# zrlhahaha/Direct12PBRRenderer

Hardware: AMD Instinct MI355X
Metric: shaded Mpixel/s at 4K G-buffer (full deferred frame: clustered shade + bloom + auto-exposure + ACES) (higher is better)
Workload: dtype f32

## Files before the change

direct12pbrrenderer_amd/csrc/exposure.hip:

```cpp
#include "pbr_internal.hpp"
#include "pbr_device.hpp"

using namespace pbr;

__device__ __forceinline__ uint32_t luminance_bin(float r, float g, float b, float min_log, float inv_range) {
#pragma clang fp contract(off)
    const float lum = (r * 0.2126f + g * 0.7152f) + b * 0.0722f;
    if (lum < EPSILON_F) return 0u;
    const float l = saturatef((log2f(lum) - min_log) * inv_range);
    return (uint32_t)floorf(l * 254.0f + 1.0f);
}

constexpr int HIST_BLOCKS = 512, HIST_NT = 1024, HIST_NW = HIST_NT / 64;

__global__ __launch_bounds__(HIST_NT) void k_lum_histogram(const pbr_half* __restrict__ hdr, uint32_t w, uint32_t h, uint32_t pitch,
                                                             float min_log, float inv_range, uint32_t* __restrict__ hist, bool vec2) {
    __shared__ uint32_t sh[HIST_NW][PBR_HISTOGRAM_BINS];
    const int wave = threadIdx.x >> 6;
    for (int i = threadIdx.x; i < HIST_NW * PBR_HISTOGRAM_BINS; i += HIST_NT) (&sh[0][0])[i] = 0u;
    __syncthreads();
    uint32_t* my = sh[wave];
    const uint32_t group = threadIdx.x >> 8, gl = threadIdx.x & 255u, stride = gridDim.x * 4u;
    if (vec2) {
        const uint32_t wp = w >> 1, upr = (wp + 255u) >> 8, units = upr * h;
        for (uint32_t u = blockIdx.x * 4u + group; u < units; u += 2 * stride) {
            const uint32_t u2 = u + stride;
            const uint32_t ya = u / upr, xa = (u - ya * upr) * 256u + gl;
            const uint32_t yb = u2 / upr, xb = (u2 - yb * upr) * 256u + gl;
            const bool ina = xa < wp, inb = u2 < units && xb < wp;
            uint4 ra = make_uint4(0u, 0u, 0u, 0u), rb = ra;
            if (ina) ra = *reinterpret_cast<const uint4*>(hdr + 4 * ((size_t)ya * pitch + 2 * xa));
            if (inb) rb = *reinterpret_cast<const uint4*>(hdr + 4 * ((size_t)yb * pitch + 2 * xb));
            const H4 p0 = *reinterpret_cast<const H4*>(&ra.x), p1 = *reinterpret_cast<const H4*>(&ra.z);
            const H4 p2 = *reinterpret_cast<const H4*>(&rb.x), p3 = *reinterpret_cast<const H4*>(&rb.z);
            hist_count(my, luminance_bin((float)p0.x, (float)p0.y, (float)p0.z, min_log, inv_range), ina);
            hist_count(my, luminance_bin((float)p1.x, (float)p1.y, (float)p1.z, min_log, inv_range), ina);
            hist_count(my, luminance_bin((float)p2.x, (float)p2.y, (float)p2.z, min_log, inv_range), inb);
            hist_count(my, luminance_bin((float)p3.x, (float)p3.y, (float)p3.z, min_log, inv_range), inb);
        }
    } else {
        const uint32_t upr = (w + 255u) >> 8, units = upr * h;
        for (uint32_t u = blockIdx.x * 4u + group; u < units; u += stride) {
            const uint32_t y = u / upr, x = (u - y * upr) * 256u + gl;
            const bool in = x < w;
            F4 c = f4(0.0f, 0.0f, 0.0f, 0.0f);
            if (in) c = load_h4(hdr + 4 * ((size_t)y * pitch + x));
            hist_count(my, luminance_bin(c.x, c.y, c.z, min_log, inv_range), in);
        }
    }
    __syncthreads();
    if (threadIdx.x < PBR_HISTOGRAM_BINS) {
        uint32_t s = 0;
#pragma unroll
        for (int k = 0; k < HIST_NW; k++) s += sh[k][threadIdx.x];
        if (s) atomicAdd(&hist[threadIdx.x], s);
    }
}

__device__ __forceinline__ float adapted_luminance(float* sh, const uint32_t* __restrict__ hist, uint32_t pixel_count, float min_log, float range,
                                                   float delta_time, float prev) {
#pragma clang fp contract(off)
    const uint32_t index = threadIdx.x;
    const uint32_t num_pixels = hist[index];
    sh[index] = (float)(uint32_t)(num_pixels * index);
    __syncthreads();
    for (uint32_t step = PBR_HISTOGRAM_BINS >> 1; step > 0; step >>= 1) {
        if (index < step) sh[index] += sh[index + step];
        __syncthreads();
    }
    float result = 0.0f;
    if (index == 0) {
        const float sum_value = sh[0];
        const float average_bin = sum_value / (float)(pixel_count - num_pixels);
        uint32_t bin = (average_bin == average_bin && average_bin > 0.0f)
                           ? (average_bin >= 4294967296.0f ? 0xFFFFFFFFu : (uint32_t)average_bin) : 0u;
        const float log_l = ((float)bin - 1.0f) / 254.0f;
        const float lum = exp2f(log_l * range + min_log);
        const float tt = saturatef(1.0f - expf(-delta_time * 1.6f));
        result = prev + tt * (lum - prev);
    }
    return result;
}

__global__ __launch_bounds__(256) void k_lum_average(uint32_t* __restrict__ hist, uint32_t pixel_count, float min_log, float range,
                                                       float delta_time, float* __restrict__ avg) {
    __shared__ float sh[PBR_HISTOGRAM_BINS];
    const float r = adapted_luminance(sh, hist, pixel_count, min_log, range, delta_time, avg[0]);
    hist[threadIdx.x] = 0u;
    if (threadIdx.x == 0) avg[0] = r;
}

struct AverageViews { uint32_t* hist[PBR_MAX_VIEWS]; float* avg[PBR_MAX_VIEWS]; float delta_time[PBR_MAX_VIEWS]; };
__global__ __launch_bounds__(256) void k_lum_average_views(AverageViews vs, uint32_t pixel_count, float min_log, float range) {
    __shared__ float sh[PBR_HISTOGRAM_BINS];
    uint32_t* hist = vs.hist[blockIdx.x];
    float* avg = vs.avg[blockIdx.x];
    const float r = adapted_luminance(sh, hist, pixel_count, min_log, range, vs.delta_time[blockIdx.x], avg[0]);
    hist[threadIdx.x] = 0u;
    if (threadIdx.x == 0) avg[0] = r;
}

__device__ __forceinline__ float aces1(float x) {
    const float a = 2.51f, b = 0.03f, c = 2.43f, d = 0.59f, e = 0.14f;
    return saturatef((x * (a * x + b)) * rcp(x * (c * x + d) + e));
}
__device__ __forceinline__ uint32_t tonemap_px(float r, float g, float b, float inv_den) {
    const float m[3] = {aces1(r * inv_den), aces1(g * inv_den), aces1(b * inv_den)};
    uint32_t px = 0xFF000000u;
#pragma unroll
    for (int k = 0; k < 3; k++) {
        const float gc = m[k] > 0.0f ? __builtin_amdgcn_exp2f(0.454545f * __builtin_amdgcn_logf(m[k])) : 0.0f;
        px |= (uint32_t)(saturatef(gc) * 255.0f + 0.5f) << (8 * k);
    }
    return px;
}

typedef float tm2 __attribute__((ext_vector_type(2)));
__device__ __forceinline__ tm2 aces2(tm2 x) {
    const float a = 2.51f, b = 0.03f, c = 2.43f, d = 0.59f, e = 0.14f;
    const tm2 num = x * (x * a + b), den = x * (x * c + d) + e;
    tm2 q;
    q.x = saturatef(num.x * rcp(den.x));
    q.y = saturatef(num.y * rcp(den.y));
    return q;
}
__device__ __forceinline__ void tonemap_px2(tm2 r, tm2 g, tm2 b, float inv_den, uint32_t& p0, uint32_t& p1) {
    const tm2 m[3] = {aces2(r * inv_den), aces2(g * inv_den), aces2(b * inv_den)};
    p0 = p1 = 0xFF000000u;
#pragma unroll
    for (int k = 0; k < 3; k++) {
        tm2 lg, gc;
        lg.x = __builtin_amdgcn_logf(m[k].x); lg.y = __builtin_amdgcn_logf(m[k].y);
        lg = lg * 0.454545f;
        gc.x = m[k].x > 0.0f ? __builtin_amdgcn_exp2f(lg.x) : 0.0f;
        gc.y = m[k].y > 0.0f ? __builtin_amdgcn_exp2f(lg.y) : 0.0f;
        gc.x = saturatef(gc.x); gc.y = saturatef(gc.y);
        const tm2 v = gc * 255.0f + 0.5f;
        p0 |= (uint32_t)v.x << (8 * k);
        p1 |= (uint32_t)v.y << (8 * k);
    }
}

__device__ __forceinline__ void tonemap_pixels(const pbr_half* __restrict__ hdr, uint32_t w, uint32_t h, uint32_t pitch,
                                               float avg_lum, uint32_t* __restrict__ out, uint32_t out_pitch, bool aligned) {
    const float l_max = 9.6f * avg_lum;
    const float inv_den = 1.0f / (l_max + 0.001f);
    const uint32_t wp = (w + 1) >> 1;
    const uint32_t upr = (wp + 255u) >> 8, units = upr * h;
    for (uint32_t u = blockIdx.x; u < units; u += gridDim.x) {
        const uint32_t y = u / upr, xp = (u - y * upr) * 256u + threadIdx.x;
        if (xp >= wp) continue;
        const uint32_t x = xp * 2;
        if (aligned && x + 1 < w) {
            const uint4 raw = *reinterpret_cast<const uint4*>(hdr + 4 * ((size_t)y * pitch + x));
            const H4 p0 = *reinterpret_cast<const H4*>(&raw.x);
            const H4 p1 = *reinterpret_cast<const H4*>(&raw.z);
            uint2 o;
            tm2 r2, g2, b2;
            r2.x = (float)p0.x; r2.y = (float)p1.x; g2.x = (float)p0.y; g2.y = (float)p1.y; b2.x = (float)p0.z; b2.y = (float)p1.z;
            tonemap_px2(r2, g2, b2, inv_den, o.x, o.y);
            *reinterpret_cast<uint2*>(out + (size_t)y * out_pitch + x) = o;
        } else {
            for (uint32_t xx = x; xx < min(x + 2, w); xx++) {
                const F4 c = load_h4(hdr + 4 * ((size_t)y * pitch + xx));
                out[(size_t)y * out_pitch + xx] = tonemap_px(c.x, c.y, c.z, inv_den);
            }
        }
    }
}

__global__ __launch_bounds__(256) void k_tonemap(const pbr_half* __restrict__ hdr, uint32_t w, uint32_t h, uint32_t pitch,
                                                   const float* __restrict__ avg, uint32_t* __restrict__ out, uint32_t out_pitch, bool aligned) {
    tonemap_pixels(hdr, w, h, pitch, avg[0], out, out_pitch, aligned);
}

struct TonemapViews {
    const pbr_half* hdr[PBR_MAX_VIEWS];
    const float* avg[PBR_MAX_VIEWS];
    uint32_t* out[PBR_MAX_VIEWS];
    uint32_t pitch[PBR_MAX_VIEWS], out_pitch[PBR_MAX_VIEWS];
    bool aligned[PBR_MAX_VIEWS];
};
__global__ __launch_bounds__(256) void k_tonemap_views(TonemapViews vs, uint32_t w, uint32_t h) {
    const uint32_t v = blockIdx.y;
    tonemap_pixels(vs.hdr[v], w, h, vs.pitch[v], vs.avg[v][0], vs.out[v], vs.out_pitch[v], vs.aligned[v]);
}

__global__ __launch_bounds__(256) void k_average_tonemap(const uint32_t* __restrict__ hist, uint32_t pixel_count, float min_log, float range,
                                                           float delta_time, const float* __restrict__ avg_in, float* __restrict__ avg_out,
                                                           uint32_t* __restrict__ hist_clear,
                                                           const pbr_half* __restrict__ hdr, uint32_t w, uint32_t h, uint32_t pitch,
                                                           uint32_t* __restrict__ out, uint32_t out_pitch, bool aligned) {
    __shared__ float sh[PBR_HISTOGRAM_BINS];
    __shared__ float s_avg;
    const float r = adapted_luminance(sh, hist, pixel_count, min_log, range, delta_time, avg_in[0]);
    if (threadIdx.x == 0) s_avg = r;
    if (blockIdx.x == 0) {
        if (hist_clear) hist_clear[threadIdx.x] = 0u;
        if (threadIdx.x == 0) avg_out[0] = r;
    }
    __syncthreads();
    tonemap_pixels(hdr, w, h, pitch, s_avg, out, out_pitch, aligned);
}

static unsigned tonemap_blocks(uint32_t w, uint32_t h) {
    const size_t pairs = (size_t)((w + 1) / 2) * h;
    const unsigned blocks = (unsigned)((pairs + 255) / 256);
    return blocks > 2048 ? 2048 : blocks;
}
static bool tonemap_aligned(const pbr_half* hdr, uint32_t pitch, const uint32_t* rgba8, uint32_t out_pitch) {
    return (((uintptr_t)hdr & 15u) == 0u) && (((uintptr_t)rgba8 & 7u) == 0u) && (((pitch | out_pitch) & 1u) == 0u);
}

extern "C" {

pbr_status pbr_lum_histogram(pbr_ctx* ctx, const pbr_half* hdr, uint32_t w, uint32_t h, uint32_t pitch,
                             float min_log, float inv_range, uint32_t* hist256) {
    if (!ctx) return PBR_ERR_INVALID;
    PBR_REQUIRE(ctx, hdr && hist256, "pbr_lum_histogram: null pointer");
    PBR_REQUIRE(ctx, w && h && w <= 65535 && h <= 65535 && pitch >= w, "pbr_lum_histogram: bad size");
    static const int max_blocks = pbr::knob_int("PBR_HIST_BLOCKS", HIST_BLOCKS);
    size_t n = (size_t)w * h;
    int blocks = (int)((n + 4095) / 4096);
    if (blocks > max_blocks) blocks = max_blocks;
    if (blocks < 1) blocks = 1;
    const bool vec2 = (((uintptr_t)hdr & 15u) == 0u) && (((w | pitch) & 1u) == 0u);
    hipLaunchKernelGGL(k_lum_histogram, dim3(blocks), dim3(HIST_NT), 0, ctx->stream, hdr, w, h, pitch, min_log, inv_range, hist256, vec2);
    return launched(ctx, "k_lum_histogram");
}

pbr_status pbr_lum_average(pbr_ctx* ctx, uint32_t* hist256, uint32_t pixel_count, float min_log, float range,
                           float delta_time, float* avg_inout) {
    if (!ctx) return PBR_ERR_INVALID;
    PBR_REQUIRE(ctx, hist256 && avg_inout, "pbr_lum_average: null pointer");
    hipLaunchKernelGGL(k_lum_average, dim3(1), dim3(256), 0, ctx->stream, hist256, pixel_count, min_log, range, delta_time, avg_inout);
    return launched(ctx, "k_lum_average");
}

pbr_status pbr_tonemap(pbr_ctx* ctx, const pbr_half* hdr, uint32_t w, uint32_t h, uint32_t pitch,
                       const float* avg, uint32_t* rgba8, uint32_t out_pitch) {
    if (!ctx) return PBR_ERR_INVALID;
    PBR_REQUIRE(ctx, hdr && avg && rgba8, "pbr_tonemap: null pointer");
    PBR_REQUIRE(ctx, w && h && w <= 65535 && h <= 65535 && pitch >= w && out_pitch >= w, "pbr_tonemap: bad size");
    hipLaunchKernelGGL(k_tonemap, dim3(tonemap_blocks(w, h)), dim3(256), 0, ctx->stream, hdr, w, h, pitch, avg, rgba8, out_pitch,
                       tonemap_aligned(hdr, pitch, rgba8, out_pitch));
    return launched(ctx, "k_tonemap");
}

pbr_status pbr_average_tonemap(pbr_ctx* ctx, const uint32_t* hist256, uint32_t pixel_count, float min_log, float range, float delta_time,
                               const float* avg_in, float* avg_out, uint32_t* hist_clear256,
                               const pbr_half* hdr, uint32_t w, uint32_t h, uint32_t pitch, uint32_t* rgba8, uint32_t out_pitch) {
    if (!ctx) return PBR_ERR_INVALID;
    PBR_REQUIRE(ctx, hist256 && avg_in && avg_out && hdr && rgba8, "pbr_average_tonemap: null pointer");
    PBR_REQUIRE(ctx, avg_in != avg_out && hist_clear256 != hist256, "pbr_average_tonemap: avg_out must differ from avg_in and hist_clear256 from hist256 (every block reads them)");
    PBR_REQUIRE(ctx, w && h && w <= 65535 && h <= 65535 && pitch >= w && out_pitch >= w, "pbr_average_tonemap: bad size");
    hipLaunchKernelGGL(k_average_tonemap, dim3(tonemap_blocks(w, h)), dim3(256), 0, ctx->stream, hist256, pixel_count, min_log, range, delta_time,
                       avg_in, avg_out, hist_clear256, hdr, w, h, pitch, rgba8, out_pitch, tonemap_aligned(hdr, pitch, rgba8, out_pitch));
    return launched(ctx, "k_average_tonemap");
}

pbr_status pbr_lum_average_views(pbr_ctx* ctx, const pbr_view* views, uint32_t n, uint32_t pixel_count, float min_log, float range) {
    if (!ctx) return PBR_ERR_INVALID;
    PBR_REQUIRE(ctx, views_count_ok(views, n), "pbr_lum_average_views: need 1 .. PBR_MAX_VIEWS views");
    AverageViews vs{};
    for (uint32_t i = 0; i < n; i++) {
        PBR_REQUIRE(ctx, views[i].hist256 && views[i].avg, "pbr_lum_average_views: null pointer");
        vs.hist[i] = views[i].hist256; vs.avg[i] = views[i].avg; vs.delta_time[i] = views[i].g.DeltaTime;
    }
    PBR_REQUIRE(ctx, views_disjoint(views, n, 2, [](const pbr_view& v, int k, uintptr_t& lo, uintptr_t& hi) {
                    if (k == 0) { lo = addr(v.hist256); hi = lo + PBR_HISTOGRAM_BINS * sizeof(uint32_t); }
                    else { lo = addr(v.avg); hi = lo + sizeof(float); } }),
                "pbr_lum_average_views: two views share a histogram or luminance cell");
    hipLaunchKernelGGL(k_lum_average_views, dim3(n), dim3(256), 0, ctx->stream, vs, pixel_count, min_log, range);
    return launched(ctx, "k_lum_average_views");
}

pbr_status pbr_tonemap_views(pbr_ctx* ctx, const pbr_view* views, uint32_t n, uint32_t w, uint32_t h) {
    if (!ctx) return PBR_ERR_INVALID;
    PBR_REQUIRE(ctx, views_count_ok(views, n), "pbr_tonemap_views: need 1 .. PBR_MAX_VIEWS views");
    PBR_REQUIRE(ctx, w && h && w <= 65535 && h <= 65535, "pbr_tonemap_views: bad size");
    TonemapViews vs{};
    for (uint32_t i = 0; i < n; i++) {
        const pbr_view& v = views[i];
        PBR_REQUIRE(ctx, v.hdr && v.avg && v.rgba8, "pbr_tonemap_views: null pointer");
        PBR_REQUIRE(ctx, v.hdr_pitch >= w && v.out_pitch >= w, "pbr_tonemap_views: bad size");
        vs.hdr[i] = v.hdr; vs.avg[i] = v.avg; vs.out[i] = v.rgba8; vs.pitch[i] = v.hdr_pitch; vs.out_pitch[i] = v.out_pitch;
        vs.aligned[i] = tonemap_aligned(v.hdr, v.hdr_pitch, v.rgba8, v.out_pitch);
    }
    PBR_REQUIRE(ctx, views_disjoint(views, n, 1, [&](const pbr_view& v, int, uintptr_t& lo, uintptr_t& hi) {
                    lo = addr(v.rgba8); hi = lo + ((size_t)v.out_pitch * (h - 1) + w) * sizeof(uint32_t); }),
                "pbr_tonemap_views: two views share an LDR target");
    hipLaunchKernelGGL(k_tonemap_views, dim3(tonemap_blocks(w, h), n), dim3(256), 0, ctx->stream, vs, w, h);
    return launched(ctx, "k_tonemap_views");
}

}
```

Baseline: 18440.

## Software-pipeline tonemap loads and prefetch HDR before exposure reduction

Restructures the tonemap pixel loop into a depth-2 software pipeline: the HDR load for the next work unit is issued before the current unit is evaluated, so memory latency overlaps with ALU work. In the fused average+tonemap kernel, the first HDR load is issued before the histogram-to-exposure reduction, hiding it behind that computation. Out-of-range lanes are clamped to the last full pixel pair and redundantly store that pair's result, and odd-width last columns get a separate tail loop. This costs extra registers per slot and adds more complex control flow.

```diff
diff --git a/direct12pbrrenderer_amd/csrc/exposure.hip b/direct12pbrrenderer_amd/csrc/exposure.hip
--- a/direct12pbrrenderer_amd/csrc/exposure.hip
+++ b/direct12pbrrenderer_amd/csrc/exposure.hip
@@ -1,5 +1,6 @@
 #include "pbr_internal.hpp"
 #include "pbr_device.hpp"
+#include "tonemap_schedule.hpp"
 
 using namespace pbr;
 
@@ -141,32 +142,69 @@
     }
 }
 
+constexpr int TONEMAP_DEPTH = 2;
+typedef uint32_t tm_u4 __attribute__((ext_vector_type(4)));
+struct TonemapSlot { tm_u4 raw; tms::Pos p; };
+struct TonemapPipe { TonemapSlot s[TONEMAP_DEPTH]; };
+
+__device__ __forceinline__ void tonemap_load(const pbr_half* __restrict__ hdr, const tms::Frame& f, TonemapSlot& s, tms::Pos p, tms::Pos at) {
+    s.p = p;
+    __builtin_amdgcn_sched_barrier(0);
+    s.raw = *reinterpret_cast<const tm_u4*>(hdr + 4 * tms::load_pixel(f, at));
+}
+
+__device__ __forceinline__ void tonemap_issue(TonemapPipe& pipe, const pbr_half* __restrict__ hdr, uint32_t w, uint32_t h, uint32_t pitch, bool aligned) {
+    const tms::Frame f = tms::frame(w, h, pitch);
+    if (!tms::pipelined(f, aligned)) return;
+    tms::prologue<TONEMAP_DEPTH>(f, blockIdx.x, gridDim.x, threadIdx.x, pipe.s,
+                                 [&](TonemapSlot& s, uint32_t, tms::Pos p, tms::Pos at, bool) { tonemap_load(hdr, f, s, p, at); });
+}
+
+__device__ __forceinline__ void tonemap_run(TonemapPipe& pipe, const pbr_half* __restrict__ hdr, uint32_t w, uint32_t h, uint32_t pitch,
+                                            float avg_lum, uint32_t* __restrict__ out, uint32_t out_pitch, bool aligned) {
+    const float l_max = 9.6f * avg_lum;
+    const float inv_den = 1.0f / (l_max + 0.001f);
+    const tms::Frame f = tms::frame(w, h, pitch);
+    if (tms::pipelined(f, aligned)) {
+        tms::loop<TONEMAP_DEPTH>(f, blockIdx.x, gridDim.x, threadIdx.x, pipe.s,
+            [&](TonemapSlot& s, uint32_t, tms::Pos p, tms::Pos at, bool) { tonemap_load(hdr, f, s, p, at); },
+            [&](TonemapSlot& s, uint32_t) {
+                tm_u4& raw = s.raw;
+                __builtin_amdgcn_sched_barrier(0);
+                asm volatile("" : "+v"(raw) : : "memory");
+                const uint2 lo = make_uint2(raw.x, raw.y), hi = make_uint2(raw.z, raw.w);
+                const H4 p0 = *reinterpret_cast<const H4*>(&lo);
+                const H4 p1 = *reinterpret_cast<const H4*>(&hi);
+                uint2 o;
+                tm2 r2, g2, b2;
+                r2.x = (float)p0.x; r2.y = (float)p1.x; g2.x = (float)p0.y; g2.y = (float)p1.y; b2.x = (float)p0.z; b2.y = (float)p1.z;
+                tonemap_px2(r2, g2, b2, inv_den, o.x, o.y);
+                const tms::Pos at = tms::clamp_pos(f, s.p);
+                *reinterpret_cast<uint2*>(out + (size_t)at.y * out_pitch + 2 * at.xp) = o;
+            });
+        if (w & 1u) {
+            for (uint32_t y = blockIdx.x * 256u + threadIdx.x; y < h; y += gridDim.x * 256u) {
+                const F4 c = load_h4(hdr + 4 * ((size_t)y * pitch + (w - 1)));
+                out[(size_t)y * out_pitch + (w - 1)] = tonemap_px(c.x, c.y, c.z, inv_den);
+            }
+        }
+        return;
+    }
+    for (uint32_t u = blockIdx.x; u < f.units; u += gridDim.x) {
+        const tms::Pos p = tms::unit_pos(f, u, threadIdx.x);
+        if (p.xp >= f.wp) continue;
+        for (uint32_t xx = p.xp * 2; xx < min(p.xp * 2 + 2, w); xx++) {
+            const F4 c = load_h4(hdr + 4 * ((size_t)p.y * pitch + xx));
+            out[(size_t)p.y * out_pitch + xx] = tonemap_px(c.x, c.y, c.z, inv_den);
+        }
+    }
+}
+
 __device__ __forceinline__ void tonemap_pixels(const pbr_half* __restrict__ hdr, uint32_t w, uint32_t h, uint32_t pitch,
                                                float avg_lum, uint32_t* __restrict__ out, uint32_t out_pitch, bool aligned) {
-    const float l_max = 9.6f * avg_lum;
-    const float inv_den = 1.0f / (l_max + 0.001f);
-    const uint32_t wp = (w + 1) >> 1;
-    const uint32_t upr = (wp + 255u) >> 8, units = upr * h;
-    for (uint32_t u = blockIdx.x; u < units; u += gridDim.x) {
-        const uint32_t y = u / upr, xp = (u - y * upr) * 256u + threadIdx.x;
-        if (xp >= wp) continue;
-        const uint32_t x = xp * 2;
-        if (aligned && x + 1 < w) {
-            const uint4 raw = *reinterpret_cast<const uint4*>(hdr + 4 * ((size_t)y * pitch + x));
-            const H4 p0 = *reinterpret_cast<const H4*>(&raw.x);
-            const H4 p1 = *reinterpret_cast<const H4*>(&raw.z);
-            uint2 o;
-            tm2 r2, g2, b2;
-            r2.x = (float)p0.x; r2.y = (float)p1.x; g2.x = (float)p0.y; g2.y = (float)p1.y; b2.x = (float)p0.z; b2.y = (float)p1.z;
-            tonemap_px2(r2, g2, b2, inv_den, o.x, o.y);
-            *reinterpret_cast<uint2*>(out + (size_t)y * out_pitch + x) = o;
-        } else {
-            for (uint32_t xx = x; xx < min(x + 2, w); xx++) {
-                const F4 c = load_h4(hdr + 4 * ((size_t)y * pitch + xx));
-                out[(size_t)y * out_pitch + xx] = tonemap_px(c.x, c.y, c.z, inv_den);
-            }
-        }
-    }
+    TonemapPipe pipe;
+    tonemap_issue(pipe, hdr, w, h, pitch, aligned);
+    tonemap_run(pipe, hdr, w, h, pitch, avg_lum, out, out_pitch, aligned);
 }
 
 __global__ __launch_bounds__(256) void k_tonemap(const pbr_half* __restrict__ hdr, uint32_t w, uint32_t h, uint32_t pitch,
@@ -193,6 +231,8 @@
                                                            uint32_t* __restrict__ out, uint32_t out_pitch, bool aligned) {
     __shared__ float sh[PBR_HISTOGRAM_BINS];
     __shared__ float s_avg;
+    TonemapPipe pipe;
+    tonemap_issue(pipe, hdr, w, h, pitch, aligned);
     const float r = adapted_luminance(sh, hist, pixel_count, min_log, range, delta_time, avg_in[0]);
     if (threadIdx.x == 0) s_avg = r;
     if (blockIdx.x == 0) {
@@ -200,7 +240,7 @@
         if (threadIdx.x == 0) avg_out[0] = r;
     }
     __syncthreads();
-    tonemap_pixels(hdr, w, h, pitch, s_avg, out, out_pitch, aligned);
+    tonemap_run(pipe, hdr, w, h, pitch, s_avg, out, out_pitch, aligned);
 }
 
 static unsigned tonemap_blocks(uint32_t w, uint32_t h) {
diff --git a/direct12pbrrenderer_amd/csrc/tonemap_schedule.hpp b/direct12pbrrenderer_amd/csrc/tonemap_schedule.hpp
--- /dev/null
+++ b/direct12pbrrenderer_amd/csrc/tonemap_schedule.hpp
@@ -0,0 +1,89 @@
+#pragma once
+#include <stddef.h>
+#include <stdint.h>
+
+#if defined(__HIPCC__)
+#define TMS_FN __host__ __device__ __forceinline__
+#define TMS_UNROLL _Pragma("unroll")
+#else
+#define TMS_FN inline
+#define TMS_UNROLL
+#endif
+
+namespace pbr {
+namespace tms {
+
+constexpr uint32_t LANES = 256;
+
+struct Frame {
+    uint32_t w, h, pitch;
+    uint32_t wp;
+    uint32_t wfull;
+    uint32_t upr, units;
+};
+TMS_FN Frame frame(uint32_t w, uint32_t h, uint32_t pitch) {
+    Frame f;
+    f.w = w; f.h = h; f.pitch = pitch;
+    f.wp = (w + 1) >> 1;
+    f.wfull = w >> 1;
+    f.upr = (f.wp + LANES - 1) / LANES;
+    f.units = f.upr * h;
+    return f;
+}
+
+struct Pos { uint32_t y, xp; };
+TMS_FN Pos unit_pos(const Frame& f, uint32_t u, uint32_t lane) {
+    Pos p;
+    p.y = u / f.upr;
+    p.xp = (u - p.y * f.upr) * LANES + lane;
+    return p;
+}
+
+TMS_FN bool pipelined(const Frame& f, bool aligned) { return aligned && f.wfull != 0u; }
+
+TMS_FN size_t load_pixel(const Frame& f, Pos p) { return (size_t)p.y * f.pitch + 2u * p.xp; }
+
+TMS_FN Pos clamp_pos(const Frame& f, Pos p) {
+    if (p.xp >= f.wfull) p.xp = f.wfull - 1u;
+    return p;
+}
+
+template <class Slot, class Load>
+TMS_FN void fill(const Frame& f, uint32_t u, uint32_t fallback, uint32_t lane, Slot& s, Load&& load) {
+    const bool exists = u < f.units;
+    const uint32_t last = f.units - 1u;
+    const Pos p = unit_pos(f, exists ? u : (fallback < last ? fallback : last), lane);
+    load(s, u, p, clamp_pos(f, p), exists && p.xp < f.wfull);
+}
+
+template <int DEPTH, class Slot, class Load>
+TMS_FN void prologue(const Frame& f, uint32_t block, uint32_t grid, uint32_t lane, Slot (&s)[DEPTH], Load&& load) {
+    static_assert(DEPTH >= 2, "one load ahead at the least");
+TMS_UNROLL
+    for (int k = 0; k < DEPTH - 1; k++) fill(f, block + (uint32_t)k * grid, block, lane, s[k], load);
+}
+
+template <int DEPTH, class Slot, class Load, class Eval>
+TMS_FN void loop(const Frame& f, uint32_t block, uint32_t grid, uint32_t lane, Slot (&s)[DEPTH], Load&& load, Eval&& eval) {
+    if (block >= f.units) return;
+    const uint32_t n = (f.units - block + grid - 1u) / grid;
+    const uint32_t rounds = n / (uint32_t)DEPTH, rem = n - rounds * (uint32_t)DEPTH;
+    uint32_t u = block;
+    auto round = [&]() {
+TMS_UNROLL
+        for (int k = 0; k < DEPTH; k++) {
+            fill(f, u + (uint32_t)(DEPTH - 1) * grid, u, lane, s[(k + DEPTH - 1) % DEPTH], load);
+            eval(s[k], u);
+            u += grid;
+        }
+    };
+    if (rounds != 0u) round();
+    for (uint32_t r = 1; r < rounds; r++) round();
+TMS_UNROLL
+    for (int k = 0; k < DEPTH - 1; k++) {
+        if ((uint32_t)k < rem) eval(s[k], u + (uint32_t)k * grid);
+    }
+}
+
+}
+}
```

After: 18410. No clear change (-0.2%).
